# jameshball/kidney-diffusion

Hardware: AMD Instinct MI355X
Metric: denoising-steps/sec (64->256 SR UNet, bs16) (higher is better)
Workload: dtype f32

## Files before the change

### include/kd_engine.h

```cpp
#ifndef KD_ENGINE_H
#define KD_ENGINE_H

#include <stddef.h>
#include <stdint.h>

#ifdef __cplusplus
extern "C" {
#endif

#define KD_MAX_LEVELS 8

const char* kd_last_error(void);
#define KD_ENGINE_ABI_VERSION 2
int kd_version(void);
const char* kd_build_id(void);

typedef struct kd_unet_config {
  int dim;
  int num_levels;
  int dim_mults[KD_MAX_LEVELS];
  int num_resnet_blocks[KD_MAX_LEVELS];
  int layer_attns[KD_MAX_LEVELS];
  int layer_cross_attns[KD_MAX_LEVELS];
  int cond_dim;
// ... 216 lines not shown

int kd_edm_sample_loop(kd_unet_t* u, const kd_edm_schedule_t* sched, const kd_sample_args_t* args, float* d_img,
                       void* stream);
int kd_edm_sample_steps(kd_unet_t* u, const kd_edm_schedule_t* sched, const kd_sample_args_t* args, float* d_img,
                        int k_begin, int k_end, void* stream);


int kd_unet_poison_scratch(kd_unet_t* u, uint32_t word, int64_t* bytes_filled, void* stream);

int kd_conv2d_nhwc(const float* d_x, const float* d_w_oihw, const float* d_bias, float* d_y,
                   int B, int Hi, int Wi, int Cin, int Cout, int KH, int KW, int stride, int pad,
                   int act, void* stream);
int kd_upsample_nearest_conv3x3_nhwc(const float* d_x, const float* d_w_oihw, const float* d_bias, float* d_y, int ldy, int yoff,
                                     int B, int H, int W, int Cin, int Cout, void* stream);
int kd_upsample_nearest_gn_conv3x3_nhwc(const float* d_x, int ldx, const float* d_ab, const float* d_w_oihw, const float* d_bias,
                                        float* d_y, int ldy, int yoff, int B, int H, int W, int Cin, int Cout, int scale,
                                        void* stream);
int kd_conv3x3_winograd_nhwc(const float* d_x, const float* d_w_oihw, const float* d_bias, float* d_y,
                             int B, int H, int W, int Cin, int Cout, void* stream);
int kd_conv3x3_winograd4_nhwc(const float* d_x, const float* d_w_oihw, const float* d_bias, const float* d_res,
                              float* d_y, int B, int H, int W, int Cin, int Cout, int G, float eps,
                              float* d_out_stats, int gemm_bf16x3, void* stream);
int kd_gemm_bf16x3(const float* d_a, const float* d_b, float* d_c, int G, int M, int N, int K, int a_planes, void* stream);
int kd_linear_bf16x3(const float* d_x, int ldx, const float* d_w, const float* d_bias, const float* d_res, int ldres,
                     const float* d_gate_src, int ldgs, const float* d_gate, int hw, float* d_y, int ldy, int M, int N, int K,
                     int act, int pixshuf_wo, double* d_seg, void* stream);
int kd_linear_bf16x3_seg_rows(int M, int N, int K);
int kd_downsample_bf16x3(const float* d_x, int ldx, const float* d_w, const float* d_bias, float* d_y, int B, int H, int W, int C,
                         int O, double* d_seg, void* stream);
int kd_gn_conv3x3_winograd_fused_nhwc(const float* d_x, const float* d_gamma, const float* d_beta,
                                      const float* d_scale_shift, const float* d_w_oihw,
                                      const float* d_bias, const float* d_res, float* d_y, int B, int H,
                                      int W, int Cin, int Cout, int G, float eps, float* d_out_stats,
                                      int ldx, void* stream);

int kd_linear_skinny(const float* d_x, int ldx, const float* d_w, const float* d_bias, float* d_y, int ldy, int M, int K,
                     int N, int in_act, int act, void* stream);
int kd_global_context_gate(const float* d_x, int B, int HW, int C, const float* d_wk, const float* d_bk, const float* d_w0,
                           const float* d_b0, int hid, const float* d_w2, const float* d_b2, float* d_gate, float* d_pooled,
                           int path, void* stream);
int kd_gate_add_nhwc(const float* d_a, const float* d_gate, const float* d_r, int ldr, float* d_y, int ldy, double* d_seg,
                     int B, int HW, int C, void* stream);
int kd_gate_add_chunks(int B, int HW);
int kd_conv_launch_shape(const int* geom, unsigned has, unsigned al16, int cus, int* out);
int kd_linattn_chunk_tokens(void);
int kd_linattn_dwconv_nhwc(const float* d_x, const float* d_wq, const float* d_wk, const float* d_wv, float* d_y,
// ... 120 lines not shown
```

### kidney-diffusion_amd/csrc/api.inc

```
extern "C" {

const char* kd_last_error(void) { return kd::g_err.c_str(); }
int kd_version(void) { return KD_ENGINE_ABI_VERSION; }

int kd_unet_create(const kd_unet_config_t* cfg, const kd_param_t* params, int n_params, kd_unet_t** out) {
  return kd_unet_create_shared(cfg, params, n_params, nullptr, out);
}

int kd_unet_create_shared(const kd_unet_config_t* cfg, const kd_param_t* params, int n_params,
                          const kd_unet_t* share_with, kd_unet_t** out) {
  return kd_unet_create_self_cond(cfg, params, n_params, share_with, 0, out);
}

int kd_unet_create_self_cond(const kd_unet_config_t* cfg, const kd_param_t* params, int n_params,
                             const kd_unet_t* share_with, int self_cond, kd_unet_t** out) {
  kd_unet_ext_t ext;
  memset(&ext, 0, sizeof ext);
  ext.self_cond = self_cond;
  return kd_unet_create_ext(cfg, params, n_params, share_with, &ext, out);
}

int kd_unet_create_ext(const kd_unet_config_t* cfg, const kd_param_t* params, int n_params, const kd_unet_t* share_with,
                       const kd_unet_ext_t* ext, kd_unet_t** out) {
  return kd_unet_create_ext2(cfg, params, n_params, share_with, ext, nullptr, out);
// ... 395 lines not shown

int kd_sample_finalize(kd_unet_t* u, const kd_sample_args_t* args, float* d_img, void* stream) {
  if (!u || !args || !d_img) {
    set_error("kd_sample_finalize: null argument");
    return 1;
  }
  return launch_finalize(d_img, args->d_inpaint_images, args->d_inpaint_masks, u->cfg.batch, u->cfg.channels,
                         (int64_t)u->cfg.image_size * u->cfg.image_size, (hipStream_t)stream);
}

namespace {
using EntryBufs = kd::DevBufs;
int entry_finish(int rc, hipStream_t s) {
  hipError_t e = hipStreamSynchronize(s);
  if (rc) return rc;
  KD_HIP_CHECK(e);
  return 0;
}
int entry_x3_ws(EntryBufs& bufs, void** ws, hipStream_t s) {
  if (bufs.get(ws, gemm_bf16x3_workspace_bytes())) return 1;
  KD_HIP_CHECK(hipMemsetAsync(*ws, 0xFF, gemm_bf16x3_workspace_bytes(), s));
  return 0;
}
X3Shape entry_x3_shape(int G, int64_t M, int N, int K) { return gemm_bf16x3_shape(G, (int)M, N, K, gemm_bf16x3_device_cus()); }
int entry_conv(const ConvParams& p, hipStream_t s) {
  return launch_conv_igemm(p, conv_shape(p, conv_ptrs_of(p), gemm_bf16x3_device_cus()), s);
}
}

int kd_conv2d_nhwc(const float* d_x, const float* d_w_oihw, const float* d_bias, float* d_y, int B, int Hi, int Wi,
                   int Cin, int Cout, int KH, int KW, int stride, int pad, int act, void* stream) {
  hipStream_t s = (hipStream_t)stream;
  const bool rowrun = (act & 0x100) != 0;
  const bool pixshuf = (act & 0x200) != 0;
  act &= 0xff;
  KD_REQUIRE(!pixshuf || (KH == 1 && KW == 1 && Cout % 4 == 0 && !rowrun), "pixel-shuffle test path: 1x1 conv, Cout % 4 == 0");
  EntryBufs bufs;
  float *wp = nullptr, *part = nullptr, *bp = nullptr;
  if (bufs.get(&wp, (size_t)Cout * Cin * KH * KW * sizeof(float))) return 1;
  if (pixshuf && bufs.get(&bp, (size_t)Cout * sizeof(float))) return 1;
  int rc = pixshuf  ? launch_pack_shuffle(d_w_oihw, d_bias, wp, bp, Cout / 4, Cin, s)
           : rowrun ? launch_pack_oihw_rowrun(d_w_oihw, wp, Cout, Cin, Cin, KH, KW, s)
                    : launch_pack_oihw(d_w_oihw, wp, Cout, Cin, Cin, KH, KW, s);
  if (!rc) {
    ConvParams p{};
    p.x = d_x; p.w = wp; p.bias = d_bias; p.y = d_y;
    p.B = B; p.Hi = Hi; p.Wi = Wi; p.Cin = Cin; p.ldx = Cin;
// ... 91 lines not shown
  KD_REQUIRE(H % 4 == 0 && W % 4 == 0, "Winograd F(4x4,3x3) path needs H % 4 == 0 and W % 4 == 0");
  const int64_t Mt = (int64_t)B * (H / 4) * (W / 4);
  KD_REQUIRE(!gemm_bf16x3 || gemm_bf16x3_ok(36, Mt, Cout, Cin),
             "bf16x3 position GEMMs need B*H*W/16 % 256 == 0, Cout % 128 == 0, Cin % 32 == 0");
  KD_REQUIRE(Mt % 128 == 0 && Cin % 32 == 0 && Cout % 64 == 0,
             "Winograd F(4x4,3x3) path needs B*H*W/16 % 128 == 0, Cin % 32 == 0, Cout % 64 == 0");
  KD_REQUIRE(!d_out_stats || (G > 0 && Cout % G == 0 && (Cout / G) % 16 == 0), "output statistics need (Cout / G) % 16 == 0");
  EntryBufs bufs;
  float *U = nullptr, *V = nullptr, *D = nullptr;
  double* seg = nullptr;
  void *U3 = nullptr, *x3ws = nullptr;
  const int nchunk = (H / 4) * (W / 4);
  if (bufs.get(&U, (size_t)36 * Cout * Cin * sizeof(float))) return 1;
  if (bufs.get(&V, (size_t)36 * Mt * Cin * (gemm_bf16x3 == 1 ? 6 : sizeof(float)))) return 1;
  if (bufs.get(&D, (size_t)36 * Mt * Cout * sizeof(float))) return 1;
  if (gemm_bf16x3 && bufs.get(&U3, (size_t)36 * Cout * Cin * 6)) return 1;
  if (gemm_bf16x3 && entry_x3_ws(bufs, &x3ws, s)) return 1;
  if (d_out_stats && bufs.get(&seg, (size_t)B * (Cout / 16) * nchunk * 2 * sizeof(double))) return 1;
  int rc = launch_wino4_pack(d_w_oihw, U, Cout, Cin, s);
  if (!rc && gemm_bf16x3) {
    rc = launch_split3(U, U3, 36, Cout, Cin, s);
    if (!rc && gemm_bf16x3 == 1) rc = launch_wino4_in3(d_x, Cin, nullptr, nullptr, nullptr, nullptr, 0, V, B, H, W, Cin, 1, s);
    if (!rc && gemm_bf16x3 != 1) rc = launch_wino4_in(d_x, Cin, nullptr, nullptr, nullptr, nullptr, 0, V, B, H, W, Cin, 1, s);
    if (!rc) rc = launch_gemm_bf16x3(V, U3, D, 36, (int)Mt, Cout, Cin, entry_x3_shape(36, Mt, Cout, Cin), x3ws, s, gemm_bf16x3 != 1);
  }
  if (!rc && !gemm_bf16x3) rc = launch_wino4_in(d_x, Cin, nullptr, nullptr, nullptr, nullptr, 0, V, B, H, W, Cin, 1, s);
  if (!rc && !gemm_bf16x3) {
    ConvParams p{};
    p.x = V; p.w = U; p.y = D;
    p.B = 1; p.Hi = 1; p.Wi = (int)(36 * Mt); p.Cin = Cin; p.ldx = Cin;
    p.Ho = 1; p.Wo = (int)(36 * Mt); p.Cout = Cout;
    p.KH = 1; p.KW = 1; p.stride = 1; p.pad = 0;
    p.out_mode = OUT_NHWC; p.ldy = Cout;
    p.wz_rows = (int)Mt; p.wz_count = 36;
    rc = entry_conv(p, s);
  }
  if (!rc) rc = launch_wino4_out(D, d_bias, d_res, Cout, d_y, Cout, seg, B, H, W, Cout, s);
  if (!rc && seg)
    rc = launch_gn_finalize(seg, d_out_stats, (Cout / G / 16) * nchunk, B, G, (double)H * W * (Cout / G), eps, s);
  return entry_finish(rc, s);
}

int kd_gemm_bf16x3(const float* d_a, const float* d_b, float* d_c, int G, int M, int N, int K, int a_planes, void* stream) {
  hipStream_t s = (hipStream_t)stream;
  KD_REQUIRE(gemm_bf16x3_ok(G, M, N, K), "kd_gemm_bf16x3 needs M % 256 == 0, N % 128 == 0, K % 32 == 0, operand planes < 4 GB");
  EntryBufs bufs;
  void *A3 = nullptr, *B3 = nullptr, *ws = nullptr;
  if (bufs.get(&B3, (size_t)G * N * K * 6)) return 1;
  if (a_planes && bufs.get(&A3, (size_t)G * M * K * 6)) return 1;
  if (entry_x3_ws(bufs, &ws, s)) return 1;
  int rc = a_planes ? launch_split3(d_a, A3, G, M, K, s) : 0;
  if (!rc) rc = launch_split3(d_b, B3, G, N, K, s);
  if (!rc) rc = launch_gemm_bf16x3(a_planes ? A3 : (const void*)d_a, B3, d_c, G, M, N, K, entry_x3_shape(G, M, N, K), ws, s, !a_planes);
  return entry_finish(rc, s);
}

int kd_downsample_bf16x3(const float* d_x, int ldx, const float* d_w, const float* d_bias, float* d_y, int B, int H, int W, int C,
                         int O, double* d_seg, void* stream) {
  hipStream_t s = (hipStream_t)stream;
  const int K = 4 * C;
  const int64_t M = (int64_t)B * (H / 2) * (W / 2);
  X3Epi e;
  e.bias = d_bias;
  e.lda = ldx > 0 ? ldx : C;
  e.ldy = O;
  e.a_tap_c = C;
  e.a_wi = W;
  e.a_hi = H;
  e.hw = (H / 2) * (W / 2);
  e.seg = d_seg;
  e.seg_nseg = d_seg ? O / 16 : 0;
  const X3Shape sh = entry_x3_shape(1, M, O, K);
  KD_REQUIRE(H > 0 && W > 0 && !(H & 1) && !(W & 1) && M < 0x7fffffff && gemm_bf16x3_epi_ok(M, O, K, e, sh),
             "kd_downsample_bf16x3 needs even map sides, C % 16 == 0, B (H/2) (W/2) % 256 == 0, O % 128 == 0");
  EntryBufs bufs;
  float *wt = nullptr, *wk = nullptr;
// ... 634 lines not shown
```

### kidney-diffusion_amd/csrc/common.h

```cpp
#pragma once
#include <hip/hip_runtime.h>
#include <stdint.h>
#include <stdio.h>
#include <algorithm>
#include <string>

#ifdef KD_EXPERIMENT
#include "../../scratch/experiment_switch.h"
#else
constexpr int kd_switch(const char*, int dflt) { return dflt; }
#endif

namespace kd {

void set_error(const std::string& msg);

#define KD_HIP_CHECK(expr)                                                               \
  do {                                                                                   \
    hipError_t _e = (expr);                                                              \
    if (_e != hipSuccess) {                                                              \
      ::kd::set_error(std::string(#expr) + " failed: " + hipGetErrorString(_e) + " at " + \
                      __FILE__ + ":" + std::to_string(__LINE__));                        \
      return 1;                                                                          \
    }                                                                                    \
// ... 98 lines not shown
}
bool gemm_bf16x3_ok(int G, int64_t M, int N, int K);
int launch_split3(const float* x, void* planes, int G, int R, int K, hipStream_t s);
size_t gemm_bf16x3_workspace_bytes();
struct X3Epi {
  const float* bias = nullptr;
  const float* res = nullptr;
  const float* gate_src = nullptr;
  const float* gate = nullptr;
  int ldres = 0, ldgs = 0;
  int hw = 0;
  int ldy = 0;
  int lda = 0;
  int a_tap_c = 0, a_wi = 0, a_hi = 0;
  double* seg = nullptr;
  int seg_nseg = 0, seg_coff = 0;
  int seg_rows8 = 0;
  int wide = 0;
  int act = ACT_NONE;
  int pixshuf_wo = 0;
};
struct X3Shape {
  int P, R, S, first;
  bool needs_sum() const { return R && S > 1; }
  int seg_rows() const { return needs_sum() ? 8 : 32; }
};
X3Shape gemm_bf16x3_shape(int G, int M, int N, int K, int cus);
int gemm_bf16x3_device_cus();
bool gemm_bf16x3_epi_ok(int64_t M, int N, int K, const X3Epi& e, const X3Shape& sh);
int launch_gemm_bf16x3(const void* A3, const void* B3, float* C, int G, int M, int N, int K, const X3Shape& sh, void* ws, hipStream_t s,
                       bool a_f32 = false, bool with_sum = true, const X3Epi* epi = nullptr);
int launch_gemm_bf16x3_sum(float* C, int G, int M, int N, int K, const X3Shape& sh, const void* ws, hipStream_t s, const X3Epi* epi = nullptr);
int launch_wino4_in3(const float* x, int ldx, const float* stats, const float* gamma, const float* beta,
                     const float* scale_shift, int ld_ss, void* V3, int B, int H, int W, int C, int G, hipStream_t s,
                     int mul_c0 = -1, float mul = 1.0f);

constexpr float WF_AB_SCALE = -1.4426950408889634f;
constexpr float WF_U_SCALE = -0.6931471805599453f;
int launch_gn_fold(const float* stats, const float* gamma, const float* beta, const float* scale_shift, int ld_ss,
                   float* ab, int B, int C, int G, hipStream_t s);
bool wino_fused128_ok(int B, int H, int W, int C, int N);
int launch_wino_fused128_pack(const float* w_oihw, float* U, int O, int I, hipStream_t s, float scale);
size_t wino_fused128_items_count(int B, int H, int W, int N);
int launch_wino_fused128_items(void* items, int B, int H, int W, int N, hipStream_t s);
size_t wino_fused_out_stats_chunks(int H, int W, int N, int G);
int launch_wino_fused_gn128(const float* x, int ldx, const float* ab, const float* U, const float* bias, const float* res,
                            int ldres, float* y, int B, int H, int W, int C, int N, double* out_partial, int out_groups,
                            const void* items, int cus, hipStream_t s);
int wino_fused_gn_max_cin();
int launch_gn_finalize(const double* partial, float* stats, int chunks, int B, int G, double count, float eps,
// ... 201 lines not shown
```

### kidney-diffusion_amd/csrc/engine.hip

```cpp
#include <stdlib.h>
#include <string.h>

#include <algorithm>
#include <cstddef>
#include <functional>
#include <map>
#include <memory>
#include <stdexcept>
#include <string>
#include <type_traits>
#include <unordered_map>
#include <unordered_set>
#include <vector>

#include "../../include/kd_engine.h"
#include "common.h"

namespace kd {

static thread_local std::string g_err;
void set_error(const std::string& msg) { g_err = msg; }

#define KD_THROW_IF(expr)                                          \
  do {                                                             \
// ... 585 lines not shown
    e.hw = x.H * x.W;
    e.act = o.act;
    e.pixshuf_wo = o.out_mode == OUT_PIXSHUF ? x.W : 0;
    return x3_epi_layer_ok(x.rows(), Cout, x.C, 128, e);
  }
  int x3_linear_images(const T& x, int Cout, int K, int stride, int pad, const ConvOpt& o) const {
    const bool whole = x3_linear_ok(x, Cout, K, stride, pad, o);
    const int cap = cfg.wino4_max_images > 0 && whole ? cfg.wino4_max_images : x.B;
    if (whole && cap >= x.B) return x.B;
    if (x.B < 2 || x.x3p || cfg.x3_linear != 0) return whole ? x.B : 0;
    for (int ns = 2; ns <= x.B; ++ns) {
      if (x.B % ns) continue;
      T xs = x;
      xs.B = x.B / ns;
      if (xs.B <= cap && x3_linear_ok(xs, Cout, K, stride, pad, o)) return xs.B;
    }
    return whole ? x.B : 0;
  }
  template <class EpiOf>
  void emit_x3_gemm(Ref a, const void* W3, Ref c, int G, int64_t M, int N, int K, bool a_f32, EpiOf epi_of,
                    const std::string& stem, const std::string& shape, int64_t macs) {
    constexpr bool has_epi = !std::is_same<EpiOf, std::nullptr_t>::value;
    if (!u->x3_ws) KD_HIP_THROW(hipMalloc(&u->x3_ws, gemm_bf16x3_workspace_bytes()));
    const X3Shape sh = gemm_bf16x3_shape(G, (int)M, N, K, u->cus);
    void* const x3_ws = u->x3_ws;
    auto launch = [=](hipStream_t s, bool sum) {
      X3Epi e;
      const X3Epi* ep = nullptr;
      if constexpr (has_epi) {
        e = epi_of();
        ep = &e;
      }
      if (sum) return launch_gemm_bf16x3_sum(c.f(), G, (int)M, N, K, sh, x3_ws, s, ep);
      return launch_gemm_bf16x3(a.f(), W3, c.f(), G, (int)M, N, K, sh, x3_ws, s, a_f32, false, ep);
    };
    emit([=](hipStream_t s) { return launch(s, false); }, stem + (has_epi ? " x3" : " gemm bf16x3") + shape, macs);
    u->macs += macs;
    u->op_mfma.back() = 6 * G * M * N * K;
    u->mfma_bf16_macs += u->op_mfma.back();
    if (sh.needs_sum()) emit([=](hipStream_t s) { return launch(s, true); }, stem + " x3 sum" + shape);
  }
  T conv(const T& x, const float* w, const float* bias, int Cout, int K, int stride, int pad, const ConvOpt& o) {
    if (x.x3p && !x3_linear_ok(x, Cout, K, stride, pad, o))
      throw std::runtime_error("plan: a tensor in plane form reached a layer that is not a bf16x3 GEMM");
    int Ho = (x.H + 2 * pad - K) / stride + 1, Wo = (x.W + 2 * pad - K) / stride + 1;
    T y;
    if (o.dst) {
// ... 1087 lines not shown
```

### kidney-diffusion_amd/csrc/kernels_gemm_bf16x3.hip

```cpp
#include "common.h"
#include "epilogue.h"

namespace kd {

namespace {

typedef float f32x16 __attribute__((ext_vector_type(16)));
typedef float f32x2 __attribute__((ext_vector_type(2)));
typedef short bf16x8 __attribute__((ext_vector_type(8)));
typedef __bf16 bf16x2 __attribute__((ext_vector_type(2)));
typedef int i32x4 __attribute__((ext_vector_type(4)));

constexpr int BM = 256, BN = 128, BK = X3_BK;
constexpr int ROWB = BK * 2;
constexpr int NST = 4;
constexpr int STAGE_B = 3 * (BM + BN) * ROWB;
constexpr int B_OFF = 3 * BM * ROWB;

__device__ __forceinline__ void dma16(const i32x4& rsrc, uint32_t lds_addr, uint32_t voff, uint32_t soff) {
  asm volatile("s_mov_b32 m0, %0\n\ts_nop 0\n\tbuffer_load_dwordx4 %1, %2, %3 offen lds" ::"s"(lds_addr), "v"(voff), "s"(rsrc),
               "s"(soff)
               : "memory");
}
__device__ __forceinline__ i32x4 make_rsrc(const void* base, uint32_t bytes) {
  const uint64_t a = (uint64_t)(uintptr_t)base;
  i32x4 r;
  r[0] = __builtin_amdgcn_readfirstlane((int)(uint32_t)a);
  r[1] = __builtin_amdgcn_readfirstlane((int)(uint32_t)((a >> 32) & 0xffffu));
  r[2] = __builtin_amdgcn_readfirstlane((int)bytes);
  r[3] = 0x00020000;
  return r;
}
template <int N>
__device__ __forceinline__ void wait_vm() {
  asm volatile("s_waitcnt vmcnt(%0)" ::"n"(N) : "memory");
}

}

__global__ __launch_bounds__(256) void split3_kernel(const float* __restrict__ x, uint32_t* __restrict__ planes, int64_t n2,
// ... 499 lines not shown
      f.a[0][i] = ahn[i];
      f.b[0][i] = bhn[i];
      f.b[2][i] = bln[i];
    }
  };
  __builtin_amdgcn_s_barrier();
#pragma unroll
  for (int p = 0; p < 3; ++p) {
    read_a(f, 0, p);
    read_b(f, 0, p);
  }
  int c = 0;
  for (int sg = 0; sg < nseg; ++sg) {
    const bool whole = sg < rounds;
    const int n = whole ? nk : tail_k1 - tail_k0, tile = seg_tile(sg);
    stage(c, X3Yes());
    for (int v = 1; v < n; ++v) stage(c + v, X3No());
    c += n;
    if (whole || S == 1) store_tile(tile);
    else put_slab(q);
  }
}

bool gemm_bf16x3_ok(int G, int64_t M, int N, int K) {
  return G > 0 && M > 0 && M % BM == 0 && N % BN == 0 && K % 32 == 0 && (int64_t)3 * G * M * K * 2 < ((int64_t)1 << 32) &&
         (int64_t)G * M * K * 4 < ((int64_t)1 << 32) &&
         (int64_t)3 * G * N * K * 2 < ((int64_t)1 << 32) && (M / BM) * (int64_t)(N / BN) * G * (K / BK) < 0x7fffffff &&
         (int64_t)G * M * N < ((int64_t)1 << 29);
}

template <bool EPI>
__global__ __launch_bounds__(256) void sum_slabs_kernel(const float* __restrict__ slab, float* __restrict__ C, int G, int M, int N,
                                                        int S, int first_tile, X3Epi e) {
  typedef float f32x4 __attribute__((ext_vector_type(4)));
  const int t = blockIdx.x >> 5, el = (blockIdx.x & 31) * 256 + threadIdx.x;
  const f32x4* s = (const f32x4*)(slab + (size_t)t * S * (BM * BN)) + el;
  f32x4 part[X3_MAX_SPLIT];
#pragma unroll
  for (int p = 0; p < X3_MAX_SPLIT; ++p) part[p] = s[(size_t)(p < S ? p : S - 1) * (BM * BN / 4)];
  f32x4 v = part[0];
#pragma unroll
  for (int p = 1; p < X3_MAX_SPLIT; ++p) v = p < S ? v + part[p] : v;
  const int lane = el & 63, wave = (el >> 6) & 7, r4 = (el >> 9) & 3, ij = el >> 11;
  const int mtiles = M / BM, ntiles = N / BN, tile = first_tile + t;
  const int nt = tile % ntiles, mt = (tile / ntiles) % mtiles, g = tile / (ntiles * mtiles);
  const int row = mt * BM + (wave >> 1) * 64 + (ij >> 1) * 32 + 8 * r4 + 4 * (lane >> 5);
// ... 33 lines not shown
      }
      d1 += __shfl_xor(d1, 32, 64);
      d2 += __shfl_xor(d2, 32, 64);
      if ((lane & 47) == 0) {
        const int bi = row / e.hw;
        double* o = e.seg + (((int64_t)bi * e.seg_nseg + ((col + e.seg_coff) >> 4)) * (e.hw >> 3) + ((row - bi * e.hw) >> 3)) * 2;
        o[0] = d1;
        o[1] = d2;
      }
    }
    return;
  }
#pragma unroll
  for (int k = 0; k < 4; ++k) c[(int64_t)k * N] = v[k];
}

int gemm_bf16x3_device_cus() {
  int dev = 0, n = 0;
  if (hipGetDevice(&dev) != hipSuccess || hipDeviceGetAttribute(&n, hipDeviceAttributeMultiprocessorCount, dev) != hipSuccess || n <= 0)
    n = 256;
  return n;
}

X3Shape gemm_bf16x3_shape(int G, int M, int N, int K, int cus) {
  const int tiles = (M / BM) * (N / BN) * G, nk = K / BK;
  if (tiles <= 0 || cus <= 0) return X3Shape{0, 0, 1, 0};
  auto split_of = [&](int r, int p) {
    int s = p / r;
    if (s > X3_MAX_SPLIT) s = X3_MAX_SPLIT;
    if (s > nk / 8) s = nk / 8;
    while (s > 1 && (nk % (2 * s)) != 0) --s;
    return s < 1 ? 1 : s;
  };
  if (tiles < cus) {
    const int S = split_of(tiles, cus);
    return X3Shape{tiles * S, tiles, S, 0};
  }
  const int R = tiles % cus;
  return X3Shape{cus, R, R ? split_of(R, cus) : 1, tiles - R};
}

static bool x3_shape_fits(const X3Shape& sh, int G, int M, int N) {
  const int tiles = (M / BM) * (N / BN) * G;
  if (sh.P <= 0 || sh.P > X3_MAX_WG || sh.R < 0 || sh.S < 1 || sh.S > X3_MAX_SPLIT || sh.first + sh.R != tiles) return false;
  return sh.first == 0 ? sh.P == sh.R * sh.S : sh.first % sh.P == 0 && sh.R * sh.S <= sh.P;
}

size_t gemm_bf16x3_workspace_bytes() {
  return (size_t)X3_MAX_WG * BM * BN * sizeof(float);
}

int launch_gemm_bf16x3_sum(float* C, int G, int M, int N, int K, const X3Shape& sh, const void* ws, hipStream_t s, const X3Epi* epi) {
  if (!sh.needs_sum()) return 0;
  KD_REQUIRE(x3_shape_fits(sh, G, M, N), "bf16x3 GEMM: the launch shape is not one of these dimensions");
  const dim3 grid((unsigned)(sh.R * 32));
  if (epi)
    hipLaunchKernelGGL(sum_slabs_kernel<true>, grid, dim3(256), 0, s, (const float*)ws, C, G, M, N, sh.S, sh.first, *epi);
  else
    hipLaunchKernelGGL(sum_slabs_kernel<false>, grid, dim3(256), 0, s, (const float*)ws, C, G, M, N, sh.S, sh.first, X3Epi{});
  KD_HIP_CHECK(hipGetLastError());
  return 0;
}
// ... 3 lines not shown
  if ((e.a_tap_c ? e.lda < e.a_tap_c : e.lda < K) || (e.ldy < N && !e.pixshuf_wo) || (e.lda & 3)) return false;
  if (e.a_tap_c && (K != 4 * e.a_tap_c || e.a_tap_c % BK || (e.a_wi & 1) || (e.a_hi & 1) || e.a_wi <= 0 || e.a_hi <= 0 ||
                    M % ((e.a_wi >> 1) * (int64_t)(e.a_hi >> 1)) || 4 * M * (int64_t)e.lda * 4 >= ((int64_t)1 << 32)))
    return false;
  if (M * (int64_t)e.lda * 4 >= ((int64_t)1 << 31) || M * (int64_t)e.ldy >= ((int64_t)1 << 29)) return false;
  if (e.res && (e.ldres < N || M * (int64_t)e.ldres * 4 >= ((int64_t)1 << 31))) return false;
  if (e.gate_src && (!e.gate || e.ldgs < N || e.hw <= 0 || e.hw % BM || M * (int64_t)e.ldgs * 4 >= ((int64_t)1 << 31))) return false;
  if (e.seg && (e.hw <= 0 || e.hw % 32 || M % e.hw || (e.seg_coff & 15) || e.seg_nseg <= 0)) return false;
  if (e.pixshuf_wo && (e.pixshuf_wo % 16 || M % e.pixshuf_wo || (N & 127) || e.res || e.gate_src || sh.needs_sum() ||
                       4 * M * (int64_t)e.ldy >= ((int64_t)1 << 29) || e.ldy < N / 4))
    return false;
  if (e.act < ACT_NONE || e.act > ACT_SIGMOID) return false;
  return true;
}

int launch_gemm_bf16x3(const void* A3, const void* B3, float* C, int G, int M, int N, int K, const X3Shape& sh, void* ws, hipStream_t s,
                       bool a_f32, bool with_sum, const X3Epi* epi) {
  KD_REQUIRE(gemm_bf16x3_ok(G, M, N, K), "bf16x3 GEMM needs M % 256 == 0, N % 128 == 0, K % 32 == 0 and operand planes < 4 GB");
  KD_REQUIRE((((uintptr_t)A3 | (uintptr_t)B3 | (uintptr_t)ws) & 15) == 0 && ws, "bf16x3 GEMM needs 16-byte aligned operand planes and a workspace");
  KD_REQUIRE(!epi || (G == 1 && gemm_bf16x3_epi_ok(M, N, K, *epi, sh) && (a_f32 || (epi->lda == K && !epi->a_tap_c))),
             "bf16x3 GEMM, epilogue form: G = 1, row strides >= the row, byte offsets < 2^31, one image per 256-row tile under a gate");
  const int P = sh.P, S = sh.S;
  KD_REQUIRE(x3_shape_fits(sh, G, M, N), "bf16x3 GEMM: the launch shape is not one of these dimensions, or has more workgroups than the workspace holds");
  float* slab = (float*)ws;
  X3Epi e = epi ? *epi : X3Epi{};
  e.seg_rows8 = sh.needs_sum();
  auto al16 = [](const void* q) { return ((uintptr_t)q & 15) == 0; };
  const bool plain_wide = !epi && !a_f32 && al16(C) && kd_switch("KD_X3_WIDE_STORE", 1) != 0;
  if (plain_wide) {
    e.ldy = N;
    e.lda = K;
  }
  e.wide = (epi || plain_wide) && al16(C) && e.ldy % 4 == 0 && al16(e.bias) && (!e.res || (al16(e.res) && e.ldres % 4 == 0)) &&
           (!e.gate_src || (al16(e.gate_src) && al16(e.gate) && e.ldgs % 4 == 0));
  const dim3 grid((unsigned)P), block(768);
  const uint16_t *a = (const uint16_t*)A3, *b = (const uint16_t*)B3;
  const int kind = plain_wide && e.wide ? 1 : !epi ? 0 : (e.act != ACT_NONE || e.pixshuf_wo || !e.wide) ? 2 : 1;
  const int tiles_all = (M / BM) * (N / BN) * G;
  const int stag = tiles_all / P >= 8 && K <= 256 ? kd_switch("KD_X3_STAGGER", 3) : 0;
  const int S_st = S | (stag << 8);
#define KD_X3(AF, EKIND) hipLaunchKernelGGL((gemm_bf16x3_kernel<AF, EKIND>), grid, block, 0, s, a, b, C, G, M, N, K, S_st, slab, e)
  if (kind == 0) {
    if (a_f32) KD_X3(true, 0); else KD_X3(false, 0);
  } else if (kind == 1) {
    if (a_f32) KD_X3(true, 1); else KD_X3(false, 1);
  } else {
    if (a_f32) KD_X3(true, 2); else KD_X3(false, 2);
  }
#undef KD_X3
  KD_HIP_CHECK(hipGetLastError());
  if (with_sum) return launch_gemm_bf16x3_sum(C, G, M, N, K, sh, ws, s, epi);
  return 0;
}

}
```

### kidney-diffusion_amd/imagen_pytorch/_engine.py

```python
from __future__ import annotations

import ctypes as C
import os
from pathlib import Path

KD_MAX_LEVELS = 8

_LIB_PATH = Path(__file__).resolve().parent.parent / "lib" / "libkd_engine.so"


class EngineUnavailable(RuntimeError):
    pass


class EngineError(RuntimeError):
    pass


class kd_unet_config_t(C.Structure):
    _fields_ = [
        ("dim", C.c_int),
        ("num_levels", C.c_int),
        ("dim_mults", C.c_int * KD_MAX_LEVELS),
        ("num_resnet_blocks", C.c_int * KD_MAX_LEVELS),
# ... 184 lines not shown
    "kd_sample_build_cond_table": (C.c_int, [C.c_void_p, C.POINTER(kd_schedule_t), C.POINTER(kd_sample_args_t), C.c_int,
                                             C.c_int, C.c_int, C.POINTER(C.c_int), C.c_void_p]),
    "kd_sample_finalize": (C.c_int, [C.c_void_p, C.POINTER(kd_sample_args_t), C.c_void_p, C.c_void_p]),
    "kd_sample_last": (C.c_int, [C.c_void_p, C.c_int, C.c_void_p, C.c_void_p]),
    "kd_sample_set_self_cond": (C.c_int, [C.c_void_p, C.c_void_p, C.c_void_p]),
    "kd_edm_sample_loop": (C.c_int, [C.c_void_p, C.POINTER(kd_edm_schedule_t), C.POINTER(kd_sample_args_t), C.c_void_p,
                                     C.c_void_p]),
    "kd_edm_sample_steps": (C.c_int, [C.c_void_p, C.POINTER(kd_edm_schedule_t), C.POINTER(kd_sample_args_t), C.c_void_p,
                                      C.c_int, C.c_int, C.c_void_p]),
    "kd_solver_sample_loop": (C.c_int, [C.c_void_p, C.POINTER(kd_solver_schedule_t), C.POINTER(kd_sample_args_t), C.c_void_p,
                                        C.c_void_p]),
    "kd_solver_sample_steps": (C.c_int, [C.c_void_p, C.POINTER(kd_solver_schedule_t), C.POINTER(kd_sample_args_t), C.c_void_p,
                                         C.c_int, C.c_int, C.c_void_p]),
    "kd_solver3_sample_loop": (C.c_int, [C.c_void_p, C.POINTER(kd_solver3_schedule_t), C.POINTER(kd_sample_args_t), C.c_void_p,
                                         C.c_void_p]),
    "kd_solver3_sample_steps": (C.c_int, [C.c_void_p, C.POINTER(kd_solver3_schedule_t), C.POINTER(kd_sample_args_t), C.c_void_p,
                                          C.c_int, C.c_int, C.c_void_p]),
    "kd_conv2d_nhwc": (C.c_int, [C.c_void_p] * 4 + [C.c_int] * 10 + [C.c_void_p]),
    "kd_upsample_nearest_conv3x3_nhwc": (C.c_int, [C.c_void_p] * 4 + [C.c_int] * 7 + [C.c_void_p]),
    "kd_upsample_nearest_gn_conv3x3_nhwc": (C.c_int, [C.c_void_p, C.c_int] + [C.c_void_p] * 4 + [C.c_int] * 8 + [C.c_void_p]),
    "kd_conv3x3_winograd_nhwc": (C.c_int, [C.c_void_p] * 4 + [C.c_int] * 5 + [C.c_void_p]),
    "kd_conv3x3_winograd4_nhwc": (C.c_int, [C.c_void_p] * 5 + [C.c_int] * 6 + [C.c_float, C.c_void_p, C.c_int, C.c_void_p]),
    "kd_gemm_bf16x3": (C.c_int, [C.c_void_p] * 3 + [C.c_int] * 5 + [C.c_void_p]),
    "kd_linear_bf16x3": (C.c_int, [C.c_void_p, C.c_int, C.c_void_p, C.c_void_p, C.c_void_p, C.c_int, C.c_void_p, C.c_int,
                                   C.c_void_p, C.c_int, C.c_void_p, C.c_int, C.c_int, C.c_int, C.c_int, C.c_int, C.c_int, C.c_void_p,
                                   C.c_void_p]),
    "kd_linear_bf16x3_seg_rows": (C.c_int, [C.c_int, C.c_int, C.c_int]),
    "kd_downsample_bf16x3": (C.c_int, [C.c_void_p, C.c_int, C.c_void_p, C.c_void_p, C.c_void_p] + [C.c_int] * 5 + [C.c_void_p, C.c_void_p]),
    "kd_gn_conv3x3_winograd_fused_nhwc": (C.c_int, [C.c_void_p] * 8 + [C.c_int] * 6 + [C.c_float, C.c_void_p, C.c_int, C.c_void_p]),
    "kd_linattn_chunk_tokens": (C.c_int, []),
    "kd_linattn_dwconv_nhwc": (C.c_int, [C.c_void_p] * 6 + [C.c_int] * 4 + [C.c_void_p]),
    "kd_linattn_context": (C.c_int, [C.c_void_p, C.c_void_p, C.c_int, C.c_void_p, C.c_int, C.c_void_p, C.c_void_p, C.c_int,
                                     C.c_int, C.c_void_p, C.c_void_p, C.c_void_p, C.c_int, C.c_int, C.c_void_p]),
    "kd_linattn_apply": (C.c_int, [C.c_void_p, C.c_int, C.c_void_p, C.c_void_p, C.c_int, C.c_int, C.c_int, C.c_int,
                                   C.c_float, C.c_int, C.c_void_p]),
    "kd_linear_skinny": (C.c_int, [C.c_void_p, C.c_int, C.c_void_p, C.c_void_p, C.c_void_p] + [C.c_int] * 6 + [C.c_void_p]),
    "kd_global_context_gate": (C.c_int, [C.c_void_p] + [C.c_int] * 3 + [C.c_void_p] * 4 + [C.c_int] + [C.c_void_p] * 4 +
                               [C.c_int, C.c_void_p]),
    "kd_gate_add_nhwc": (C.c_int, [C.c_void_p] * 3 + [C.c_int, C.c_void_p, C.c_int, C.c_void_p] + [C.c_int] * 3 + [C.c_void_p]),
    "kd_gate_add_chunks": (C.c_int, [C.c_int, C.c_int]),
    "kd_conv_launch_shape": (C.c_int, [C.c_void_p, C.c_uint, C.c_uint, C.c_int, C.c_void_p]),
    "kd_gn_fold_seg": (C.c_int, [C.c_void_p, C.c_int, C.c_int, C.c_float, C.c_float, C.c_void_p, C.c_int, C.c_int, C.c_float,
                                 C.c_float] + [C.c_void_p] * 3 + [C.c_int] + [C.c_void_p] * 2 + [C.c_int] * 4 +
                       [C.c_float, C.c_void_p]),
    "kd_wf_ab_scale": (C.c_float, []),
    "kd_gn_conv3x3_winograd4_nhwc": (C.c_int, [C.c_void_p, C.c_int] + [C.c_void_p] * 4 + [C.c_int, C.c_int, C.c_float] +
# ... 162 lines not shown
```

Baseline: 41.24.

## Add half-tile pipelined bf16x3 GEMM kernel for fp32-A, K=128 shapes

Adds a new bf16x3 GEMM kernel that processes each 256-row tile as two 128-row halves, with a 6-stage LDS ring and producer waves that split fp32 A in flight. It overlaps one half's output stores with the next half's MFMA work. A shape rule enables it by default for fp32-A, no-epilogue GEMMs with K==128 and 2-16 rounds per CU, and an env switch controls it. The intent is to hide epilogue store latency and smooth the pipeline for short-K persistent GEMMs, at the cost of a more complex kernel and a narrower shape coverage.

```diff
diff --git a/include/kd_engine.h b/include/kd_engine.h
--- a/include/kd_engine.h
+++ b/include/kd_engine.h
@@ -262,6 +262,7 @@
                               float* d_y, int B, int H, int W, int Cin, int Cout, int G, float eps,
                               float* d_out_stats, int gemm_bf16x3, void* stream);
 int kd_gemm_bf16x3(const float* d_a, const float* d_b, float* d_c, int G, int M, int N, int K, int a_planes, void* stream);
+int kd_gemm_bf16x3_form(const float* d_a, const float* d_b, float* d_c, int G, int M, int N, int K, int halves, void* stream);
 int kd_linear_bf16x3(const float* d_x, int ldx, const float* d_w, const float* d_bias, const float* d_res, int ldres,
                      const float* d_gate_src, int ldgs, const float* d_gate, int hw, float* d_y, int ldy, int M, int N, int K,
                      int act, int pixshuf_wo, double* d_seg, void* stream);
diff --git a/kidney-diffusion_amd/csrc/api.inc b/kidney-diffusion_amd/csrc/api.inc
--- a/kidney-diffusion_amd/csrc/api.inc
+++ b/kidney-diffusion_amd/csrc/api.inc
@@ -441,7 +441,9 @@
   KD_HIP_CHECK(hipMemsetAsync(*ws, 0xFF, gemm_bf16x3_workspace_bytes(), s));
   return 0;
 }
-X3Shape entry_x3_shape(int G, int64_t M, int N, int K) { return gemm_bf16x3_shape(G, (int)M, N, K, gemm_bf16x3_device_cus()); }
+X3Shape entry_x3_shape(int G, int64_t M, int N, int K, bool a_f32_plain = false) {
+  return gemm_bf16x3_shape(G, (int)M, N, K, gemm_bf16x3_device_cus(), a_f32_plain);
+}
 int entry_conv(const ConvParams& p, hipStream_t s) {
   return launch_conv_igemm(p, conv_shape(p, conv_ptrs_of(p), gemm_bf16x3_device_cus()), s);
 }
@@ -579,7 +581,7 @@
     rc = launch_split3(U, U3, 36, Cout, Cin, s);
     if (!rc && gemm_bf16x3 == 1) rc = launch_wino4_in3(d_x, Cin, nullptr, nullptr, nullptr, nullptr, 0, V, B, H, W, Cin, 1, s);
     if (!rc && gemm_bf16x3 != 1) rc = launch_wino4_in(d_x, Cin, nullptr, nullptr, nullptr, nullptr, 0, V, B, H, W, Cin, 1, s);
-    if (!rc) rc = launch_gemm_bf16x3(V, U3, D, 36, (int)Mt, Cout, Cin, entry_x3_shape(36, Mt, Cout, Cin), x3ws, s, gemm_bf16x3 != 1);
+    if (!rc) rc = launch_gemm_bf16x3(V, U3, D, 36, (int)Mt, Cout, Cin, entry_x3_shape(36, Mt, Cout, Cin, gemm_bf16x3 != 1), x3ws, s, gemm_bf16x3 != 1);
   }
   if (!rc && !gemm_bf16x3) rc = launch_wino4_in(d_x, Cin, nullptr, nullptr, nullptr, nullptr, 0, V, B, H, W, Cin, 1, s);
   if (!rc && !gemm_bf16x3) {
@@ -608,7 +610,22 @@
   if (entry_x3_ws(bufs, &ws, s)) return 1;
   int rc = a_planes ? launch_split3(d_a, A3, G, M, K, s) : 0;
   if (!rc) rc = launch_split3(d_b, B3, G, N, K, s);
-  if (!rc) rc = launch_gemm_bf16x3(a_planes ? A3 : (const void*)d_a, B3, d_c, G, M, N, K, entry_x3_shape(G, M, N, K), ws, s, !a_planes);
+  if (!rc) rc = launch_gemm_bf16x3(a_planes ? A3 : (const void*)d_a, B3, d_c, G, M, N, K, entry_x3_shape(G, M, N, K, !a_planes), ws, s, !a_planes);
+  return entry_finish(rc, s);
+}
+
+int kd_gemm_bf16x3_form(const float* d_a, const float* d_b, float* d_c, int G, int M, int N, int K, int halves, void* stream) {
+  hipStream_t s = (hipStream_t)stream;
+  KD_REQUIRE(gemm_bf16x3_ok(G, M, N, K), "kd_gemm_bf16x3_form needs M % 256 == 0, N % 128 == 0, K % 32 == 0, operand planes < 4 GB");
+  X3Shape sh = entry_x3_shape(G, M, N, K);
+  sh.halves = halves != 0;
+  KD_REQUIRE(!sh.halves || gemm_bf16x3_halves_legal(sh, K), "kd_gemm_bf16x3_form, halves form: no tile cut in k, K >= 128");
+  EntryBufs bufs;
+  void *B3 = nullptr, *ws = nullptr;
+  if (bufs.get(&B3, (size_t)G * N * K * 6)) return 1;
+  if (entry_x3_ws(bufs, &ws, s)) return 1;
+  int rc = launch_split3(d_b, B3, G, N, K, s);
+  if (!rc) rc = launch_gemm_bf16x3(d_a, B3, d_c, G, M, N, K, sh, ws, s, true);
   return entry_finish(rc, s);
 }
 
diff --git a/kidney-diffusion_amd/csrc/common.h b/kidney-diffusion_amd/csrc/common.h
--- a/kidney-diffusion_amd/csrc/common.h
+++ b/kidney-diffusion_amd/csrc/common.h
@@ -144,10 +144,12 @@
 };
 struct X3Shape {
   int P, R, S, first;
+  int halves = 0;
   bool needs_sum() const { return R && S > 1; }
   int seg_rows() const { return needs_sum() ? 8 : 32; }
 };
-X3Shape gemm_bf16x3_shape(int G, int M, int N, int K, int cus);
+X3Shape gemm_bf16x3_shape(int G, int M, int N, int K, int cus, bool a_f32_plain = false);
+bool gemm_bf16x3_halves_legal(const X3Shape& sh, int K);
 int gemm_bf16x3_device_cus();
 bool gemm_bf16x3_epi_ok(int64_t M, int N, int K, const X3Epi& e, const X3Shape& sh);
 int launch_gemm_bf16x3(const void* A3, const void* B3, float* C, int G, int M, int N, int K, const X3Shape& sh, void* ws, hipStream_t s,
diff --git a/kidney-diffusion_amd/csrc/engine.hip b/kidney-diffusion_amd/csrc/engine.hip
--- a/kidney-diffusion_amd/csrc/engine.hip
+++ b/kidney-diffusion_amd/csrc/engine.hip
@@ -631,7 +631,7 @@
                     const std::string& stem, const std::string& shape, int64_t macs) {
     constexpr bool has_epi = !std::is_same<EpiOf, std::nullptr_t>::value;
     if (!u->x3_ws) KD_HIP_THROW(hipMalloc(&u->x3_ws, gemm_bf16x3_workspace_bytes()));
-    const X3Shape sh = gemm_bf16x3_shape(G, (int)M, N, K, u->cus);
+    const X3Shape sh = gemm_bf16x3_shape(G, (int)M, N, K, u->cus, a_f32 && !has_epi);
     void* const x3_ws = u->x3_ws;
     auto launch = [=](hipStream_t s, bool sum) {
       X3Epi e;
diff --git a/kidney-diffusion_amd/csrc/kernels_gemm_bf16x3.hip b/kidney-diffusion_amd/csrc/kernels_gemm_bf16x3.hip
--- a/kidney-diffusion_amd/csrc/kernels_gemm_bf16x3.hip
+++ b/kidney-diffusion_amd/csrc/kernels_gemm_bf16x3.hip
@@ -16,6 +16,9 @@
 constexpr int NST = 4;
 constexpr int STAGE_B = 3 * (BM + BN) * ROWB;
 constexpr int B_OFF = 3 * BM * ROWB;
+constexpr int HM = 128, NSTH = 6;
+constexpr int UNIT_B = 3 * (HM + BN) * ROWB;
+constexpr int BH_OFF = 3 * HM * ROWB;
 
 __device__ __forceinline__ void dma16(const i32x4& rsrc, uint32_t lds_addr, uint32_t voff, uint32_t soff) {
   asm volatile("s_mov_b32 m0, %0\n\ts_nop 0\n\tbuffer_load_dwordx4 %1, %2, %3 offen lds" ::"s"(lds_addr), "v"(voff), "s"(rsrc),
@@ -561,6 +564,222 @@
   }
 }
 
+__global__ __launch_bounds__(768) void gemm_bf16x3_halves_kernel(const float* __restrict__ A, const uint16_t* __restrict__ B3,
+                                                                 float* __restrict__ C, int G, int M, int N, int K, int stagger) {
+  __shared__ __attribute__((aligned(1024))) char lds[NSTH * UNIT_B];
+  const int tid = threadIdx.x, lane = tid & 63;
+  const int wave = __builtin_amdgcn_readfirstlane(tid >> 6);
+  const int mtiles = M / BM, ntiles = N / BN;
+  const int nk = K / BK;
+  const int P = gridDim.x;
+  int q = blockIdx.x;
+  if ((P & 7) == 0) q = (blockIdx.x & 7) * (P >> 3) + (blockIdx.x >> 3);
+  const int tiles = mtiles * ntiles * G, rounds = tiles / P, R = tiles - rounds * P;
+  if (stagger && (q & 1))
+    for (int i = 0; i < stagger; ++i) __builtin_amdgcn_s_sleep(127);
+  const int nseg = rounds + (q < R ? 1 : 0);
+  const int T = nseg * 2 * nk;
+  const uint32_t lds0 = (uint32_t)(uintptr_t)(__attribute__((address_space(3))) char*)lds;
+  if (wave >= 8) {
+    const int l = wave - 8;
+    const uint32_t planeB = (uint32_t)((int64_t)G * N * K * 2);
+    const i32x4 rsB = make_rsrc(B3, 3u * planeB);
+    const i32x4 rsA = make_rsrc(A, (uint32_t)((int64_t)G * M * K * 4));
+    const uint32_t voffB = (uint32_t)((lane >> 1) * ROWB + (((lane & 1) ^ ((lane >> 4) & 1)) * 16));
+    const uint32_t chunkB = (uint32_t)(N * ROWB);
+    const int arow = l * 16 + (lane >> 2), aq = lane & 3;
+    constexpr int NR = 2, PER = NR + 3;
+    uint32_t voffAj[NR];
+#pragma unroll
+    for (int j = 0; j < NR; ++j) voffAj[j] = (uint32_t)(((arow + 64 * j) * K + aq * 4) * 4);
+    const int ldsA = arow * ROWB + ((((aq >> 1) ^ ((arow >> 3) & 1)) * 16) + (aq & 1) * 8);
+    int ic = 0, iseg = 0, ih = 0, ik = 0;
+    uint32_t baseA = 0, baseB = 0;
+    auto locate = [&]() __attribute__((always_inline)) {
+      const int it = iseg * P + q;
+      const int nt = it % ntiles, mt = (it / ntiles) % mtiles, g = it / (ntiles * mtiles);
+      baseA = (uint32_t)(((int64_t)g * M + mt * BM + ih * HM) * K * 4);
+      baseB = (uint32_t)((int64_t)g * N * K * 2) + (uint32_t)(nt * BN * ROWB);
+    };
+    locate();
+    typedef unsigned int u32x4 __attribute__((ext_vector_type(4)));
+    typedef unsigned int u32x2 __attribute__((ext_vector_type(2)));
+    u32x4 ra[NSTH][NR];
+    auto issue_next = [&](auto SET) __attribute__((always_inline)) {
+      constexpr int set = decltype(SET)::value;
+      const uint32_t soA = baseA + (uint32_t)(ik * (BK * 4));
+#pragma unroll
+      for (int j = 0; j < NR; ++j)
+        asm volatile("buffer_load_dwordx4 %0, %1, %2, %3 offen" : "=&v"(ra[set][j]) : "v"(voffAj[j]), "s"(rsA), "s"(soA) : "memory");
+#pragma unroll
+      for (int j = 0; j < 3; ++j) {
+        const int id = l * 3 + j, pl = id >> 2, pr = id & 3;
+        const uint32_t dst = lds0 + (uint32_t)(set * UNIT_B + BH_OFF + (pl * BN + pr * 32) * ROWB);
+        dma16(rsB, dst, voffB, (uint32_t)pl * planeB + baseB + (uint32_t)ik * chunkB + (uint32_t)(pr * 32 * ROWB));
+      }
+      ++ic;
+      if (++ik == nk) {
+        ik = 0;
+        if (++ih == 2) {
+          ih = 0;
+          ++iseg;
+        }
+        if (ic < T) locate();
+      }
+    };
+    auto wait_a = [&](int u, u32x4(&r)[NR]) __attribute__((always_inline)) {
+      if (ic < u + NSTH - 1) asm volatile("s_waitcnt vmcnt(0)" ::: "memory");
+      asm volatile("s_waitcnt vmcnt(%2)" : "+v"(r[0]), "+v"(r[1]) : "n"(3 + (NSTH - 2) * PER) : "memory");
+    };
+    auto wait_b = [&](int u) __attribute__((always_inline)) {
+      if (ic < u + NSTH - 1) wait_vm<0>(); else wait_vm<(NSTH - 2) * PER>();
+    };
+    auto write_unit = [&](int u, auto SET) __attribute__((always_inline)) {
+      constexpr int set = decltype(SET)::value;
+      wait_a(u, ra[set]);
+      char* dst = lds + set * UNIT_B + ldsA;
+#pragma unroll
+      for (int j = 0; j < NR; ++j) {
+        uint32_t h0, m0, l0, h1, m1, l1;
+        const f32x2 v01 = {__uint_as_float(ra[set][j][0]), __uint_as_float(ra[set][j][1])};
+        const f32x2 v23 = {__uint_as_float(ra[set][j][2]), __uint_as_float(ra[set][j][3])};
+        x3_split(v01, h0, m0, l0);
+        x3_split(v23, h1, m1, l1);
+        *(u32x2*)(dst + j * 64 * ROWB) = u32x2{h0, h1};
+        *(u32x2*)(dst + HM * ROWB + j * 64 * ROWB) = u32x2{m0, m1};
+        *(u32x2*)(dst + 2 * HM * ROWB + j * 64 * ROWB) = u32x2{l0, l1};
+      }
+      wait_b(u);
+    };
+    if (ic < T) issue_next(X3Set<0>());
+    if (ic < T) issue_next(X3Set<1>());
+    if (ic < T) issue_next(X3Set<2>());
+    if (ic < T) issue_next(X3Set<3>());
+    if (ic < T) issue_next(X3Set<4>());
+    if (ic < T) issue_next(X3Set<5>());
+    write_unit(0, X3Set<0>());
+    asm volatile("s_waitcnt lgkmcnt(0)" ::: "memory");
+    __builtin_amdgcn_s_barrier();
+    auto iter = [&](int c, auto SET_W, auto SET_I) __attribute__((always_inline)) {
+      if (c + 1 < T) write_unit(c + 1, SET_W);
+      asm volatile("s_waitcnt lgkmcnt(0)" ::: "memory");
+      __builtin_amdgcn_s_barrier();
+      if (ic < T) issue_next(SET_I);
+    };
+    for (int c = 0; c < T; c += 6) {
+      iter(c, X3Set<1>(), X3Set<0>());
+      if (c + 1 < T) iter(c + 1, X3Set<2>(), X3Set<1>());
+      if (c + 2 < T) iter(c + 2, X3Set<3>(), X3Set<2>());
+      if (c + 3 < T) iter(c + 3, X3Set<4>(), X3Set<3>());
+      if (c + 4 < T) iter(c + 4, X3Set<5>(), X3Set<4>());
+      if (c + 5 < T) iter(c + 5, X3Set<0>(), X3Set<5>());
+    }
+    return;
+  }
+  const int wm = wave >> 1, wn = wave & 1;
+  const f32x16 zero16 = {0.f, 0.f, 0.f, 0.f, 0.f, 0.f, 0.f, 0.f, 0.f, 0.f, 0.f, 0.f, 0.f, 0.f, 0.f, 0.f};
+  f32x16 accX[2], accY[2] = {zero16, zero16};
+  const int fr = lane & 31, fh = lane >> 5;
+  const int fslot = (fh ^ ((fr >> 3) & 1)) * 16;
+  const char* fa = lds + (wm * 32 + fr) * ROWB + fslot;
+  const char* fb = lds + BH_OFF + (wn * 64 + fr) * ROWB + fslot;
+  const int vC = ((wm * 32 + 4 * fh) * N + wn * 64 + fr) * 4;
+  bf16x8 fa3[3], fb3[3][2], ahn, bhn[2], bln[2];
+  int so = 0;
+  auto store_slice = [&](auto SLICE, const f32x16(&old)[2], __amdgpu_buffer_rsrc_t rs, int s0) __attribute__((always_inline)) {
+    constexpr int sl = decltype(SLICE)::value, j = sl >> 2, r4 = sl & 3;
+    int Nv = N;
+    asm volatile("" : "+s"(Nv));
+#pragma unroll
+    for (int k = 0; k < 4; ++k)
+      __builtin_amdgcn_raw_buffer_store_b32(__float_as_uint(old[j][4 * r4 + k]), rs, vC, s0 + ((8 * r4 + k) * Nv + j * 32) * 4, 0);
+  };
+  auto stage = [&](auto FRESH, auto SLICE, f32x16(&acc)[2], const f32x16(&old)[2], __amdgpu_buffer_rsrc_t rs, int s0)
+                   __attribute__((always_inline)) {
+    __builtin_amdgcn_s_barrier();
+    const f32x16 zero = {0.f, 0.f, 0.f, 0.f, 0.f, 0.f, 0.f, 0.f, 0.f, 0.f, 0.f, 0.f, 0.f, 0.f, 0.f, 0.f};
+#pragma unroll
+    for (int j = 0; j < 2; ++j)
+      acc[j] = __builtin_amdgcn_mfma_f32_32x32x16_bf16(fa3[2], fb3[0][j], decltype(FRESH)::value ? zero : acc[j], 0, 0, 0);
+    __builtin_amdgcn_sched_barrier(0);
+    fa3[2] = *(const bf16x8*)(fa + so + 2 * HM * ROWB);
+    ahn = *(const bf16x8*)(fa + so);
+#pragma unroll
+    for (int j = 0; j < 2; ++j) {
+      bhn[j] = *(const bf16x8*)(fb + so + j * 32 * ROWB);
+      bln[j] = *(const bf16x8*)(fb + so + 2 * BN * ROWB + j * 32 * ROWB);
+    }
+    __builtin_amdgcn_sched_barrier(0);
+#pragma unroll
+    for (int j = 0; j < 2; ++j) acc[j] = __builtin_amdgcn_mfma_f32_32x32x16_bf16(fa3[1], fb3[0][j], acc[j], 0, 0, 0);
+    if constexpr (decltype(SLICE)::value >= 0) {
+      __builtin_amdgcn_sched_barrier(0);
+      store_slice(SLICE, old, rs, s0);
+      __builtin_amdgcn_sched_barrier(0);
+    }
+#pragma unroll
+    for (int j = 0; j < 2; ++j) acc[j] = __builtin_amdgcn_mfma_f32_32x32x16_bf16(fa3[1], fb3[1][j], acc[j], 0, 0, 0);
+    __builtin_amdgcn_sched_barrier(0);
+    fa3[1] = *(const bf16x8*)(fa + so + HM * ROWB);
+    __builtin_amdgcn_sched_barrier(0);
+#pragma unroll
+    for (int j = 0; j < 2; ++j) acc[j] = __builtin_amdgcn_mfma_f32_32x32x16_bf16(fa3[0], fb3[0][j], acc[j], 0, 0, 0);
+#pragma unroll
+    for (int j = 0; j < 2; ++j) acc[j] = __builtin_amdgcn_mfma_f32_32x32x16_bf16(fa3[0], fb3[1][j], acc[j], 0, 0, 0);
+    __builtin_amdgcn_sched_barrier(0);
+#pragma unroll
+    for (int j = 0; j < 2; ++j) fb3[1][j] = *(const bf16x8*)(fb + so + BN * ROWB + j * 32 * ROWB);
+    __builtin_amdgcn_sched_barrier(0);
+#pragma unroll
+    for (int j = 0; j < 2; ++j) acc[j] = __builtin_amdgcn_mfma_f32_32x32x16_bf16(fa3[0], fb3[2][j], acc[j], 0, 0, 0);
+    fa3[0] = ahn;
+#pragma unroll
+    for (int j = 0; j < 2; ++j) {
+      fb3[0][j] = bhn[j];
+      fb3[2][j] = bln[j];
+    }
+    so = so == (NSTH - 1) * UNIT_B ? 0 : so + UNIT_B;
+  };
+  auto half = [&](f32x16(&acc)[2], const f32x16(&old)[2], __amdgpu_buffer_rsrc_t rs, int s0) __attribute__((always_inline)) {
+    stage(X3Yes(), X3Set<0>(), acc, old, rs, s0);
+    stage(X3No(), X3Set<1>(), acc, old, rs, s0);
+    stage(X3No(), X3Set<2>(), acc, old, rs, s0);
+    stage(X3No(), X3Set<3>(), acc, old, rs, s0);
+    stage(X3No(), X3Set<4>(), acc, old, rs, s0);
+    stage(X3No(), X3Set<5>(), acc, old, rs, s0);
+    stage(X3No(), X3Set<6>(), acc, old, rs, s0);
+    stage(X3No(), X3Set<7>(), acc, old, rs, s0);
+    for (int v = 8; v < nk; ++v) stage(X3No(), X3Set<-1>(), acc, old, rs, s0);
+  };
+  const int c_bytes = (int)((int64_t)G * M * N * 4);
+  const __amdgpu_buffer_rsrc_t rsC = __builtin_amdgcn_make_buffer_rsrc((void*)C, 0, c_bytes, 0x00020000);
+  __builtin_amdgcn_s_barrier();
+#pragma unroll
+  for (int p = 0; p < 3; ++p) {
+    fa3[p] = *(const bf16x8*)(fa + p * HM * ROWB);
+#pragma unroll
+    for (int j = 0; j < 2; ++j) fb3[p][j] = *(const bf16x8*)(fb + p * BN * ROWB + j * 32 * ROWB);
+  }
+  so = UNIT_B;
+  int s_y = 0;
+  for (int sg = 0; sg < nseg; ++sg) {
+    const int tile = sg * P + q;
+    const int nt = tile % ntiles, mt = (tile / ntiles) % mtiles, g = tile / (ntiles * mtiles);
+    const int s_x = ((g * M + mt * BM) * N + nt * BN) * 4;
+    half(accX, accY, __builtin_amdgcn_make_buffer_rsrc((void*)C, 0, sg ? c_bytes : 0, 0x00020000), s_y);
+    s_y = s_x + HM * N * 4;
+    half(accY, accX, rsC, s_x);
+  }
+  store_slice(X3Set<0>(), accY, rsC, s_y);
+  store_slice(X3Set<1>(), accY, rsC, s_y);
+  store_slice(X3Set<2>(), accY, rsC, s_y);
+  store_slice(X3Set<3>(), accY, rsC, s_y);
+  store_slice(X3Set<4>(), accY, rsC, s_y);
+  store_slice(X3Set<5>(), accY, rsC, s_y);
+  store_slice(X3Set<6>(), accY, rsC, s_y);
+  store_slice(X3Set<7>(), accY, rsC, s_y);
+}
+
 bool gemm_bf16x3_ok(int G, int64_t M, int N, int K) {
   return G > 0 && M > 0 && M % BM == 0 && N % BN == 0 && K % 32 == 0 && (int64_t)3 * G * M * K * 2 < ((int64_t)1 << 32) &&
          (int64_t)G * M * K * 4 < ((int64_t)1 << 32) &&
@@ -640,7 +859,7 @@
   return n;
 }
 
-X3Shape gemm_bf16x3_shape(int G, int M, int N, int K, int cus) {
+static X3Shape x3_whole_shape(int G, int M, int N, int K, int cus) {
   const int tiles = (M / BM) * (N / BN) * G, nk = K / BK;
   if (tiles <= 0 || cus <= 0) return X3Shape{0, 0, 1, 0};
   auto split_of = [&](int r, int p) {
@@ -656,6 +875,23 @@
   }
   const int R = tiles % cus;
   return X3Shape{cus, R, R ? split_of(R, cus) : 1, tiles - R};
+}
+
+bool gemm_bf16x3_halves_legal(const X3Shape& sh, int K) { return !sh.needs_sum() && K >= 8 * BK; }
+
+static bool x3_halves_rule(const X3Shape& sh, int G, int M, int N, int K) {
+  const int mode = kd_switch("KD_X3_HALVES", 1);
+  if (!gemm_bf16x3_halves_legal(sh, K) || mode == 0) return false;
+  if (mode == 2) return true;
+  const int tiles = (M / BM) * (N / BN) * G;
+  const int rounds = tiles / sh.P;
+  return K == 128 && rounds >= 2 && rounds <= 16;
+}
+
+X3Shape gemm_bf16x3_shape(int G, int M, int N, int K, int cus, bool a_f32_plain) {
+  X3Shape sh = x3_whole_shape(G, M, N, K, cus);
+  sh.halves = a_f32_plain && sh.P > 0 && x3_halves_rule(sh, G, M, N, K);
+  return sh;
 }
 
 static bool x3_shape_fits(const X3Shape& sh, int G, int M, int N) {
@@ -705,6 +941,16 @@
              "bf16x3 GEMM, epilogue form: G = 1, row strides >= the row, byte offsets < 2^31, one image per 256-row tile under a gate");
   const int P = sh.P, S = sh.S;
   KD_REQUIRE(x3_shape_fits(sh, G, M, N), "bf16x3 GEMM: the launch shape is not one of these dimensions, or has more workgroups than the workspace holds");
+  const int tiles_all = (M / BM) * (N / BN) * G;
+  if (sh.halves) {
+    KD_REQUIRE(a_f32 && !epi && gemm_bf16x3_halves_legal(sh, K),
+               "bf16x3 GEMM, halves form: fp32 A, no epilogue, no tile cut in k, K >= 128");
+    const int stag = tiles_all / P >= 8 ? kd_switch("KD_X3_HALVES_STAGGER", 0) : 0;
+    hipLaunchKernelGGL(gemm_bf16x3_halves_kernel, dim3((unsigned)P), dim3(768), 0, s, (const float*)A3, (const uint16_t*)B3, C, G, M,
+                       N, K, stag);
+    KD_HIP_CHECK(hipGetLastError());
+    return 0;
+  }
   float* slab = (float*)ws;
   X3Epi e = epi ? *epi : X3Epi{};
   e.seg_rows8 = sh.needs_sum();
@@ -719,7 +965,6 @@
   const dim3 grid((unsigned)P), block(768);
   const uint16_t *a = (const uint16_t*)A3, *b = (const uint16_t*)B3;
   const int kind = plain_wide && e.wide ? 1 : !epi ? 0 : (e.act != ACT_NONE || e.pixshuf_wo || !e.wide) ? 2 : 1;
-  const int tiles_all = (M / BM) * (N / BN) * G;
   const int stag = tiles_all / P >= 8 && K <= 256 ? kd_switch("KD_X3_STAGGER", 3) : 0;
   const int S_st = S | (stag << 8);
 #define KD_X3(AF, EKIND) hipLaunchKernelGGL((gemm_bf16x3_kernel<AF, EKIND>), grid, block, 0, s, a, b, C, G, M, N, K, S_st, slab, e)
diff --git a/kidney-diffusion_amd/imagen_pytorch/_engine.py b/kidney-diffusion_amd/imagen_pytorch/_engine.py
--- a/kidney-diffusion_amd/imagen_pytorch/_engine.py
+++ b/kidney-diffusion_amd/imagen_pytorch/_engine.py
@@ -230,6 +230,7 @@
     "kd_conv3x3_winograd_nhwc": (C.c_int, [C.c_void_p] * 4 + [C.c_int] * 5 + [C.c_void_p]),
     "kd_conv3x3_winograd4_nhwc": (C.c_int, [C.c_void_p] * 5 + [C.c_int] * 6 + [C.c_float, C.c_void_p, C.c_int, C.c_void_p]),
     "kd_gemm_bf16x3": (C.c_int, [C.c_void_p] * 3 + [C.c_int] * 5 + [C.c_void_p]),
+    "kd_gemm_bf16x3_form": (C.c_int, [C.c_void_p] * 3 + [C.c_int] * 5 + [C.c_void_p]),
     "kd_linear_bf16x3": (C.c_int, [C.c_void_p, C.c_int, C.c_void_p, C.c_void_p, C.c_void_p, C.c_int, C.c_void_p, C.c_int,
                                    C.c_void_p, C.c_int, C.c_void_p, C.c_int, C.c_int, C.c_int, C.c_int, C.c_int, C.c_int, C.c_void_p,
                                    C.c_void_p]),
```

Result: no change. 41.42 (median of 2 runs) (+0.4%).
